# SimplySnap/torchPDLP

Measured on AMD Instinct MI355X. Metric: PDHG iterations/sec, higher is better.
Workload: dtype f32; 1 GPU; synthetic random feasible LP 10000000x10000000, 100 nnz/row (density 1.0e-05), gen_lp recipe 'box' seed 0; nnz=1000000000, primal_weight_update=True, parallelism=single GPU

## Files before the change

### include/pdlp_hip.h

```cpp
#ifndef PDLP_HIP_H
#define PDLP_HIP_H

#include <stdint.h>

#ifdef __cplusplus
extern "C" {
#endif

#define PDLP_OK 0
#define PDLP_ERR_INVALID (-1)
#define PDLP_ERR_WORKSPACE (-2)
#define PDLP_ERR_STATE (-3)
#define PDLP_ERR_COMM (-4)
#define PDLP_ERR_HIP_BASE (-1000)

enum { PDLP_F32 = 0, PDLP_F64 = 1, PDLP_MIXED = 2 };

enum { PDLP_CUR = 0, PDLP_AVG = 1, PDLP_PREV = 2 };

enum {
    PDLP_BUF_X_CUR = 0, PDLP_BUF_X_PREV = 1, PDLP_BUF_XBAR = 2, PDLP_BUF_X_AVG = 3,
    PDLP_BUF_Y_CUR = 4, PDLP_BUF_Y_PREV = 5, PDLP_BUF_Y_AVG = 6,
    PDLP_BUF_RED = 7,
    PDLP_BUF_X_SUM = 8, PDLP_BUF_Y_SUM = 9,
// ... 38 lines not shown
    const int32_t* tile_ptr;
    const int64_t* blk_base;
    const uint32_t* cnt;
    int32_t rem_rows_n, rem_segs_n;
    const int32_t* rem_rows;
    const int32_t* rem_rptr;
    const int32_t* rem_sptr;
    const int32_t* rem_col;
    const void* rem_val;
    void* rem_work;
    void* rem_extra;
    void* rem_extra_f32;
} pdlp_tiles;

typedef struct pdlp_solver* pdlp_handle;

const char* pdlp_strerror(int code);
int pdlp_abi_version(void);

int pdlp_workspace_bytes(const pdlp_problem* p, int64_t* bytes);
int pdlp_create(pdlp_handle* out, const pdlp_problem* p, void* workspace, int64_t workspace_bytes);
void pdlp_destroy(pdlp_handle h);
int pdlp_attach_tiles(pdlp_handle h, int transpose, const pdlp_tiles* t);
int pdlp_schedule_info(pdlp_handle h, int transpose, int32_t* nblk, const int64_t** blocks);
int pdlp_attach_sorted(pdlp_handle h, int transpose, const uint32_t* sidx, const void* sval, const int32_t* cbase);
int pdlp_buffer_ptr(pdlp_handle h, int which, void** ptr);

int pdlp_set_iterate(pdlp_handle h, const void* x_local, const void* y_local);
int pdlp_get_iterate(pdlp_handle h, int which, void* x_local, void* y_local);
int pdlp_set_step(pdlp_handle h, double eta, double omega, double theta, int64_t iteration);
int pdlp_set_omega(pdlp_handle h, double omega);
int pdlp_get_scalars(pdlp_handle h, double out[PDLP_NSCAL]);

int pdlp_primal_half(pdlp_handle h, int adaptive);
int pdlp_dual_half(pdlp_handle h, int adaptive);
int pdlp_primal_half_begin(pdlp_handle h);
int pdlp_dual_half_begin(pdlp_handle h, int adaptive);
int pdlp_split_info(pdlp_handle h, int transpose, int32_t out[4]);
int pdlp_tile_limits(pdlp_handle h, int32_t out[6]);
int pdlp_adaptive_retry(pdlp_handle h);
int pdlp_adaptive_reduce(pdlp_handle h);
int pdlp_adaptive_update(pdlp_handle h);
int pdlp_iterate(pdlp_handle h, int iters, int adaptive);
int pdlp_fixed_advance(pdlp_handle h, int iters);
int pdlp_halpern_iterate(pdlp_handle h, int iters);

// ... 119 lines not shown
```

### torchpdlp_amd/_native.py

```python
from __future__ import annotations

import ctypes as C
import os

_HERE = os.path.dirname(os.path.abspath(__file__))
LIB_PATH = os.environ.get("PDLP_LIB") or os.path.join(_HERE, "libpdlp_hip.so")

ABI_VERSION = 18
PDLP_F32, PDLP_F64, PDLP_MIXED = 0, 1, 2
CUR, AVG, PREV = 0, 1, 2
(BUF_X_CUR, BUF_X_PREV, BUF_XBAR, BUF_X_AVG, BUF_Y_CUR, BUF_Y_PREV, BUF_Y_AVG, BUF_RED, BUF_X_SUM, BUF_Y_SUM,
 BUF_SCALARS, BUF_DX, BUF_DY, BUF_LAM_PREV, BUF_GDX, BUF_GDY) = range(16)
NRED, NSCAL = 8, 16
OPT_RUNNING_KKT, OPT_KTY_REUSE, OPT_GRAPH, OPT_SPLIT_SLOTS, OPT_PRODUCER_PIECES, OPT_BEGIN_INLINE, OPT_PEER_EXCHANGE, OPT_PEER_TIMEOUT_MS, OPT_PEER_LOCAL_FIRST, OPT_PEER_PUSH = range(10)
PEER_INFO_BYTES, PEER_LOOPBACK, PEER_LOOPBACK_HOST = 256, 1, 2
S_ETA, S_OMEGA, S_THETA, S_TAU, S_SIGMA, S_WPEND, S_ETASUM, S_K, S_INV1PT, S_ACCEPT, S_ETABAR, S_DEN, S_ETASUM_PREV = range(13)


class PdlpProblem(C.Structure):
    _fields_ = [("dtype", C.c_int32), ("device", C.c_int32), ("m", C.c_int64), ("n", C.c_int64), ("m_ineq", C.c_int64),
                ("row0", C.c_int64), ("row1", C.c_int64), ("col0", C.c_int64), ("col1", C.c_int64),
                ("K_rowptr", C.c_void_p), ("K_colidx", C.c_void_p), ("K_val", C.c_void_p),
                ("KT_rowptr", C.c_void_p), ("KT_colidx", C.c_void_p), ("KT_val", C.c_void_p),
                ("c", C.c_void_p), ("l", C.c_void_p), ("u", C.c_void_p), ("q", C.c_void_p),
# ... 18 lines not shown
                ("dy", C.c_void_p),
                ("eta", C.c_void_p), ("omega", C.c_void_p), ("eta_sum", C.c_void_p), ("wpend", C.c_void_p),
                ("live", C.c_void_p), ("action", C.c_void_p), ("part", C.c_void_p), ("out", C.c_void_p)]


class PdlpBatchFeed(C.Structure):
    _fields_ = [("N", C.c_int32), ("c", C.c_void_p), ("q", C.c_void_p), ("l", C.c_void_p), ("u", C.c_void_p),
                ("x0", C.c_void_p), ("y0", C.c_void_p), ("K_val", C.c_void_p), ("KT_val", C.c_void_p),
                ("eta", C.c_void_p), ("omega", C.c_void_p)]


BATCH_PART_PER_COL = 2 * 4 * 8192


_H = C.c_void_p
_I, _I64, _D, _P = C.c_int, C.c_int64, C.c_double, C.c_void_p
SIGNATURES = {
    "pdlp_strerror": (C.c_char_p, [_I]),
    "pdlp_abi_version": (_I, []),
    "pdlp_workspace_bytes": (_I, [C.POINTER(PdlpProblem), C.POINTER(_I64)]),
    "pdlp_create": (_I, [C.POINTER(_H), C.POINTER(PdlpProblem), _P, _I64]),
    "pdlp_destroy": (None, [_H]),
    "pdlp_attach_tiles": (_I, [_H, _I, C.POINTER(PdlpTiles)]),
    "pdlp_schedule_info": (_I, [_H, _I, C.POINTER(C.c_int32), C.POINTER(_P)]),
    "pdlp_attach_sorted": (_I, [_H, _I, _P, _P, _P]),
    "pdlp_buffer_ptr": (_I, [_H, _I, C.POINTER(_P)]),
    "pdlp_set_iterate": (_I, [_H, _P, _P]),
    "pdlp_get_iterate": (_I, [_H, _I, _P, _P]),
    "pdlp_set_step": (_I, [_H, _D, _D, _D, _I64]),
    "pdlp_set_omega": (_I, [_H, _D]),
    "pdlp_get_scalars": (_I, [_H, C.POINTER(_D)]),
    "pdlp_primal_half": (_I, [_H, _I]),
    "pdlp_dual_half": (_I, [_H, _I]),
    "pdlp_primal_half_piece": (_I, [_H, _I, _I, _I]),
    "pdlp_dual_half_piece": (_I, [_H, _I, _I, _I]),
    "pdlp_primal_half_begin": (_I, [_H]),
    "pdlp_dual_half_begin": (_I, [_H, _I]),
    "pdlp_split_info": (_I, [_H, _I, C.POINTER(C.c_int32)]),
    "pdlp_tile_limits": (_I, [_H, C.POINTER(C.c_int32)]),
    "pdlp_adaptive_retry": (_I, [_H]),
    "pdlp_adaptive_reduce": (_I, [_H]),
    "pdlp_adaptive_update": (_I, [_H]),
    "pdlp_iterate": (_I, [_H, _I, _I]),
    "pdlp_halpern_iterate": (_I, [_H, _I]),
    "pdlp_set_row_upper": (_I, [_H, _P]),
    "pdlp_set_exchange_chunks": (_I, [_H, _I]),
# ... 117 lines not shown
```

### torchpdlp_amd/csrc/pdlp_handle.inc

```
namespace {

struct Schedule {
    int64_t* blk = nullptr;
    uint32_t* rplo = nullptr;
    int nblk = 0;
    int grid = 0;
    int64_t* lch = nullptr;
    int32_t* lrow = nullptr;
    int32_t* lptr = nullptr;
    void* longpart = nullptr;
    int nchunks = 0, nlong = 0, lgrid = 0;
    const uint32_t* sidx = nullptr;
    const void* sval = nullptr;
    const int32_t* cbase = nullptr;
    bool tiled = false;
    pdlp_tiles t{};
    int loc_pa = 0, loc_pb = 0;
    int slotsA = 0, slotsB = 0;
    bool pending = false;
    bool pending_inline = false;
    int32_t* ptab = nullptr;
    int64_t ptab_cap = 0;
    int nphase = 0;
    int ph_off[MAX_PHASE] = {0}, ph_cnt[MAX_PHASE] = {0}, ph_slots[MAX_PHASE] = {0}, ph_slot0[MAX_PHASE] = {0};
    int64_t sb[MAX_PHASE] = {0};
    int chunks_done = 0;
    int nrange = 0;
    int rb_lo[MAX_PHASE] = {0};
};

inline int64_t max_blocks(int64_t rows, int64_t nnz) { return 2 * (rows / ROWS_CAP + nnz / NNZ_CAP) + 4; }

inline int64_t max_chunks(int64_t nnz) { return 2 * (nnz / NNZ_CAP) + 2; }
inline int64_t max_long(int64_t nnz) { return nnz / NNZ_CAP + 1; }
constexpr int LONG_GRID = 64;

inline int64_t rowsum_groups(int64_t rows)
{
    if (rows <= (int64_t)512 * 40 * 128) return 32;
// ... 267 lines not shown
```

### torchpdlp_amd/csrc/pdlp_hip.hip

```cpp
#include <hip/hip_runtime.h>
#include <rccl/rccl.h>
#include <dlfcn.h>
#include <unistd.h>

#include <cmath>
#include <cstdint>
#include <cstdio>
#include <cstdlib>
#include <cstring>
#include <new>
#include <type_traits>
#include <vector>

#include "pdlp_hip.h"

namespace {

constexpr int BLOCK = 256;
constexpr int NNZ_CAP = 2048;
constexpr int ROWS_CAP = 256;
constexpr int MAX_GRID = 2048;
constexpr int NACC = 4;
constexpr int MAX_CHUNKS = 4;
constexpr int MAX_PHASE = MAX_CHUNKS + 2;
// ... 165 lines not shown
        case PDLP_BUF_X_AVG: *ptr = h->xb[h->ix_avg]; break;
        case PDLP_BUF_Y_CUR: *ptr = h->yb[h->ix_cur]; break;
        case PDLP_BUF_Y_PREV: *ptr = h->yb[h->ix_prev]; break;
        case PDLP_BUF_Y_AVG: *ptr = h->yb[h->ix_avg]; break;
        case PDLP_BUF_RED: *ptr = h->red; break;
        case PDLP_BUF_X_SUM: *ptr = h->x_sum; break;
        case PDLP_BUF_Y_SUM: *ptr = h->y_sum; break;
        case PDLP_BUF_SCALARS: *ptr = h->sc; break;
        case PDLP_BUF_DX: *ptr = h->dxf; break;
        case PDLP_BUF_DY: *ptr = h->dyf; break;
        case PDLP_BUF_LAM_PREV: *ptr = h->lam_prev; break;
        case PDLP_BUF_GDX: if (!h->mixed) return PDLP_ERR_STATE; *ptr = h->gdx; break;
        case PDLP_BUF_GDY: if (!h->mixed) return PDLP_ERR_STATE; *ptr = h->gdy; break;
        default: return PDLP_ERR_INVALID;
    }
    return PDLP_OK;
}

int pdlp_attach_tiles(pdlp_handle h, int transpose, const pdlp_tiles* t)
{
    if (!h) return PDLP_ERR_INVALID;
    Schedule& s = transpose ? h->sKT : h->sK;
    drop_graphs(h);
    if (!t) { s.tiled = false; return configure_split(h, transpose != 0); }
    const int64_t rows = transpose ? h->nl : h->ml;
    const int rpt_max = h->p.dtype == PDLP_F64 ? TileCfg<double, double>::RPT_MAX : TileCfg<float, float>::RPT_MAX;
    const int cap_max = h->p.dtype == PDLP_F64 ? TileCfg<double, double>::CAP : TileCfg<float, float>::CAP;
    if (t->rpt < 1 || t->rpt > rpt_max || t->cap > cap_max || t->lw < 4 || (((uint64_t)t->cap + 8u) << t->lw) > (1ull << 32)) return PDLP_ERR_INVALID;
    const int64_t rb = (int64_t)TNT * t->rpt;
    if (t->nblk != (int)((rows + rb - 1) / rb) || t->npanel < 1) return PDLP_ERR_INVALID;
    if (t->groups < 1 || t->groups > h->rs_groups || t->groups > t->npanel) return PDLP_ERR_INVALID;
    if (t->nblk > h->part_blocks) return PDLP_ERR_INVALID;
    if (!t->idx || !t->val || !t->tile_ptr || !t->blk_base || !t->cnt) return PDLP_ERR_INVALID;
    if (((uintptr_t)t->idx & 15u) || ((uintptr_t)t->val & 15u) || ((uintptr_t)t->cnt & 15u)) return PDLP_ERR_INVALID;
    if (t->rem_rows_n < 0 || t->rem_segs_n < t->rem_rows_n) return PDLP_ERR_INVALID;
    if (t->rem_rows_n > 0 && (!t->rem_rows || !t->rem_rptr || !t->rem_sptr || !t->rem_col || !t->rem_val || !t->rem_work || !t->rem_extra ||
                              (h->mixed && !t->rem_extra_f32)))
        return PDLP_ERR_INVALID;
    s.t = *t;
    s.tiled = true;
    return configure_split(h, transpose != 0);
}

int pdlp_schedule_info(pdlp_handle h, int transpose, int32_t* nblk, const int64_t** blocks)
{
    if (!h || !nblk || !blocks) return PDLP_ERR_INVALID;
    const Schedule& s = transpose ? h->sKT : h->sK;
    *nblk = s.nblk;
    *blocks = s.blk;
    return PDLP_OK;
}

int pdlp_attach_sorted(pdlp_handle h, int transpose, const uint32_t* sidx, const void* sval, const int32_t* cbase)
{
    if (!h) return PDLP_ERR_INVALID;
    if ((sidx == nullptr) != (sval == nullptr) || (sidx == nullptr) != (cbase == nullptr)) return PDLP_ERR_INVALID;
    Schedule& s = transpose ? h->sKT : h->sK;
    drop_graphs(h);
    s.sidx = sidx; s.sval = sval; s.cbase = cbase;
    return PDLP_OK;
}

int pdlp_set_iterate(pdlp_handle h, const void* x_local, const void* y_local)
{
// ... 376 lines not shown
```

### torchpdlp_amd/csrc/pdlp_kernel_tiled.inc

```
#ifndef PDLP_PRIO_P1
#define PDLP_PRIO_P1 3
#define PDLP_PRIO_P2 0
#endif
#ifndef PDLP_GROUP_FAST
#define PDLP_GROUP_FAST 1
#endif
#ifndef PDLP_EPI_GROUP
#define PDLP_EPI_GROUP 0
#endif
#ifndef PDLP_TNT
#define PDLP_TNT 512
#endif
constexpr int TNT = PDLP_TNT;
typedef unsigned int u32x4 __attribute__((ext_vector_type(4)));
typedef float f32x4 __attribute__((ext_vector_type(4)));
typedef double f64x4 __attribute__((ext_vector_type(4)));
#ifndef PDLP_F32_RPT
#define PDLP_F32_RPT 40
#define PDLP_F32_CAP 16384
#define PDLP_F32_TU 4
#endif
template <typename T, typename TV> struct TileCfg;
template <> struct TileCfg<float, float> { static constexpr int RPT_MAX = PDLP_F32_RPT, CAP = PDLP_F32_CAP, TU = PDLP_F32_TU, MINW = 4; typedef f32x4 V4; };
template <> struct TileCfg<double, double> { static constexpr int RPT_MAX = 24, CAP = 8192, TU = 2, MINW = 4; typedef f64x4 V4; };
template <> struct TileCfg<double, float> { static constexpr int RPT_MAX = PDLP_F32_RPT, CAP = PDLP_F32_CAP > 16384 ? 16384 : PDLP_F32_CAP, TU = 2, MINW = 2; typedef f32x4 V4; };
constexpr int TRPT_MAX_ANY = PDLP_F32_RPT > 40 ? PDLP_F32_RPT : 40;

__device__ __forceinline__ float fma_t(float a, float b, float c) { return __builtin_fmaf(a, b, c); }
__device__ __forceinline__ double fma_t(double a, double b, double c) { return __builtin_fma(a, b, c); }
__device__ __forceinline__ float clamp01_t(float x) { return __builtin_amdgcn_fmed3f(x, 0.0f, 1.0f); }
__device__ __forceinline__ double clamp01_t(double x) { return __builtin_fmin(__builtin_fmax(x, 0.0), 1.0); }

template <typename T, typename TV, class Epi, bool FUSED>
__global__ __launch_bounds__(TNT, (TileCfg<T, TV>::MINW)) void k_tiled_fused(const uint32_t* __restrict__ tidx, const TV* __restrict__ tval,
                                                        const int32_t* __restrict__ tile_ptr, const int64_t* __restrict__ blk_base,
                                                        const uint32_t* __restrict__ tcnt,
                                                        int npanel, int lw, int rpt, int nrows, int nblk,
                                                        int vtotal, const int32_t* __restrict__ ptab, int slot0, int b0, int nbl,
                                                        const T* __restrict__ vin, T* __restrict__ rowsum,
                                                        int64_t rs_stride, const T* __restrict__ extra, Epi epi,
                                                        double* __restrict__ partials)
{
    typedef TileCfg<T, TV> Cfg;
    constexpr int TRPT_MAX = Cfg::RPT_MAX, TCW = TRPT_MAX / 8, TCAP = Cfg::CAP, TU = Cfg::TU;
    constexpr int TGRP = TNT * 4 * TU;
    typedef typename Cfg::V4 V4;
    __shared__ __attribute__((aligned(16))) T prod[TCAP + 8];
    __shared__ int wsum[TNT / 64];
    __shared__ double dred8[TNT / 64];
    const int tid = threadIdx.x, lane = tid & 63, wv = tid >> 6;
    const int ngrp = FUSED ? 1 : (int)(gridDim.x / (unsigned)nbl);
#if PDLP_GROUP_FAST
    const int b = FUSED ? blockIdx.x : b0 + (int)(blockIdx.x / (unsigned)ngrp);
    const int grp = FUSED ? 0 : (int)(blockIdx.x % (unsigned)ngrp);
#else
    const int b = FUSED ? blockIdx.x : b0 + (int)(blockIdx.x % (unsigned)nbl);
    const int grp = FUSED ? 0 : (int)(blockIdx.x / (unsigned)nbl);
#endif
    const int p_lo = (int)((int64_t)grp * vtotal / ngrp), p_hi = (int)((int64_t)(grp + 1) * vtotal / ngrp);
    auto pmap = [&](int v) { return ptab ? ptab[v] : v; };
    const uint32_t mask = (1u << lw) - 1u;
    if (FUSED) epi.load();
    T acc[TRPT_MAX];
#pragma unroll
    for (int r = 0; r < TRPT_MAX; ++r) acc[r] = (T)0;

    const uint32_t trash = (uint32_t)TCAP << lw;
    tidx += blk_base[b];
    tval += blk_base[b];
    auto load_into = [&](u32x4 (&pk)[TU], V4 (&vv)[TU], int g0, int i1) {
#pragma unroll
        for (int u = 0; u < TU; ++u) {
            const int i = g0 + (u * TNT + tid) * 4;
            if (i < i1) {
                pk[u] = __builtin_nontemporal_load(reinterpret_cast<const u32x4*>(tidx + i));
                vv[u] = __builtin_nontemporal_load(reinterpret_cast<const V4*>(tval + i));
            } else {
                pk[u] = u32x4{trash, trash, trash, trash};
                vv[u] = V4{(TV)0, (TV)0, (TV)0, (TV)0};
            }
        }
    };
#ifndef PDLP_ROUND
#define PDLP_ROUND 4
#endif
    auto consume = [&](u32x4 (&pk)[TU], V4 (&vv)[TU], int g0, int i1, const T* __restrict__ xin) {
        constexpr int RPC = 4 / PDLP_ROUND, NR = TU * RPC;
        T xg[TU * 4];
        bool on[TU];
#pragma unroll
        for (int u = 0; u < TU; ++u) on[u] = g0 + (u * TNT + __builtin_amdgcn_readfirstlane(wv) * 64) * 4 < i1;
        auto pkw = [&](int u, int k) -> uint32_t { return k == 0 ? pk[u].x : k == 1 ? pk[u].y : k == 2 ? pk[u].z : pk[u].w; };
        auto vvw = [&](int u, int k) -> TV { return k == 0 ? vv[u].x : k == 1 ? vv[u].y : k == 2 ? vv[u].z : vv[u].w; };
        auto products = [&](int r) {
            const int u = r / RPC, k0 = (r % RPC) * PDLP_ROUND;
            if (on[u]) {
#pragma unroll
                for (int k = k0; k < k0 + PDLP_ROUND; ++k) prod[pkw(u, k) >> lw] = (T)vvw(u, k) * xg[4 * u + k];
            }
        };
#pragma unroll
        for (int r = 0; r < NR; ++r) {
            const int u = r / RPC, k0 = (r % RPC) * PDLP_ROUND;
            if (r > 0) { products(r - 1); __builtin_amdgcn_sched_barrier(0); }
            if (on[u]) {
#pragma unroll
                for (int k = k0; k < k0 + PDLP_ROUND; ++k) {
                    xg[4 * u + k] = *reinterpret_cast<const T*>(reinterpret_cast<const char*>(xin) + ((pkw(u, k) & mask) * (uint32_t)sizeof(T)));
                }
            }
            __builtin_amdgcn_sched_barrier(0);
        }
        products(NR - 1);
    };
    const size_t tile0 = (size_t)b * npanel;
    const size_t tp0 = (size_t)b * (npanel + 1);
    const bool has_panels = p_lo < vtotal;
    const size_t ntiles = (size_t)nblk * npanel;
    auto load_counts = [&](uint32_t (&cwd)[TCW], size_t tile) {
        const u32x4 a = __builtin_nontemporal_load(reinterpret_cast<const u32x4*>(tcnt) + tile * TNT + tid);
        cwd[0] = a.x;
        if (TCW > 1) cwd[1 < TCW ? 1 : 0] = a.y;
        if (TCW > 2) cwd[2 < TCW ? 2 : 0] = a.z;
        if (TCW > 3) cwd[3 < TCW ? 3 : 0] = a.w;
#pragma unroll
        for (int q = 4; q < TCW; ++q) cwd[q] = __builtin_nontemporal_load(tcnt + ntiles * TNT * 4 + (tile * (TCW > 4 ? TCW - 4 : 1) + (q - 4)) * TNT + tid);
    };
    u32x4 pk[TU];
    V4 vv[TU];
    int i0 = has_panels ? tile_ptr[tp0 + pmap(p_lo)] : 0;
    int i1 = has_panels ? tile_ptr[tp0 + pmap(p_lo) + 1] : 0;
    load_into(pk, vv, i0, i1);

    for (int i = tid; i < TCAP + 8; i += TNT) prod[i] = (T)0;
    __syncthreads();
    uint32_t cwn[TCW];
    {
        load_counts(cwn, tile0 + (has_panels ? pmap(p_lo) : 0));
    }
    for (int v = p_lo; v < p_hi; ++v) {
        const int p = pmap(v);
        const T* __restrict__ xin = vin + ((size_t)p << lw);
        int i0n = i1, i1n = i1;
        if (v + 1 < p_hi) {
            const int pn = pmap(v + 1);
            i0n = tile_ptr[tp0 + pn];
            i1n = tile_ptr[tp0 + pn + 1];
        }
        uint32_t cw[TCW];
        uint32_t total = 0;
#pragma unroll
        for (int q = 0; q < TCW; ++q) cw[q] = cwn[q];
#pragma unroll
        for (int q = 0; q < TCW; ++q) {
            const uint32_t n2 = (cw[q] & 0x0f0f0f0fu) + ((cw[q] >> 4) & 0x0f0f0f0fu);
            total += (n2 * 0x01010101u) >> 24;
        }
        total = wave_incl_scan_u32(total);
        if (lane == 63) wsum[wv] = (int)total;
        __builtin_amdgcn_s_setprio(PDLP_PRIO_P1);
        for (int g0 = i0; g0 < i1; g0 += TGRP) {
            consume(pk, vv, g0, i1, xin);
            if (g0 + TGRP < i1) load_into(pk, vv, g0 + TGRP, i1);
            else load_into(pk, vv, i0n, i1n);
        }
        if (i0 >= i1) load_into(pk, vv, i0n, i1n);
        {
            load_counts(cwn, tile0 + (v + 1 < p_hi ? pmap(v + 1) : p));
        }
        __builtin_amdgcn_s_setprio(PDLP_PRIO_P2);
        __syncthreads();
        int sb = 0;
#pragma unroll
        for (int w = 0; w < TNT / 64; ++w) sb += (w < wv) ? wsum[w] : 0;
        uint32_t sbase = (uint32_t)__builtin_amdgcn_readfirstlane(sb);
#pragma unroll
        for (int q = 0; q < TCW; ++q) {
            if (8 * q < rpt) {
                uint32_t cE = cw[q] & 0x0f0f0f0fu, cO = (cw[q] >> 4) & 0x0f0f0f0fu;
                asm("" : "+v"(cE), "+v"(cO));
                uint32_t sE = cE, sO = cO;
                wave_incl_scan2_u32(sE, sO);
                const uint32_t tE = (uint32_t)__builtin_amdgcn_readlane((int)sE, 63), tO = (uint32_t)__builtin_amdgcn_readlane((int)sO, 63);
                const uint32_t eE = sE - cE, eO = sO - cO;
                constexpr int RG = sizeof(T) == 8 ? 2 : 4;
#pragma unroll
                for (int g = 0; g < 8 / RG; ++g) {
                    if (8 * q + RG * g < rpt) {
                        int cc[RG], oo[RG];
// ... 111 lines not shown
        for (int g0 = 0; g0 < groups; g0 += 4) {
            T part[4];
#pragma unroll
            for (int k = 0; k < 4; ++k) {
                const int g = g0 + k < glast ? g0 + k : glast;
                part[k] = __builtin_nontemporal_load(rowsum + (size_t)g * rs_stride + row);
            }
            s = g0 == 0 ? part[0] : s + part[0];
#pragma unroll
            for (int k = 1; k < 4; ++k) s = g0 + k < groups ? s + part[k] : s;
        }
        if (extra) s += extra[row];
        epi(row, s, pre, acc);
    }
    if (Epi::NA > 0) {
#pragma unroll
        for (int r = 0; r < Epi::NA; ++r) {
            const double v = block_sum(acc[r], dred);
            if (threadIdx.x == 0) partials[(size_t)blockIdx.x * NACC + r] = v;
        }
    }
}

template <typename T, typename TV>
__global__ __launch_bounds__(BLOCK) void k_rem_segments(int ns, const int32_t* __restrict__ sptr, const int32_t* __restrict__ col,
                                                        const TV* __restrict__ val, const T* __restrict__ vin, T* __restrict__ seg_sum)
{
    const int lt = threadIdx.x & 7;
    const int64_t stride = ((int64_t)gridDim.x * BLOCK) >> 3;
    const int64_t ns_pad = ((int64_t)ns + stride - 1) / stride * stride;
    for (int64_t g = ((int64_t)blockIdx.x * BLOCK + threadIdx.x) >> 3; g < ns_pad; g += stride) {
        T s = (T)0;
        if (g < ns) {
            const int a = sptr[g], nn = sptr[g + 1] - a;
            const int last = nn - 1;
            for (int i0 = lt; i0 < nn; i0 += 64) {
                T lv[8], lg[8];
                int lc[8];
#pragma unroll
                for (int u = 0; u < 8; ++u) {
                    const int i = i0 + 8 * u, ic = i < last ? i : last;
                    lv[u] = (T)val[a + ic];
                    lc[u] = col[a + ic];
                }
#pragma unroll
                for (int u = 0; u < 8; ++u) lg[u] = vin[lc[u]];
// ... 49 lines not shown
```

### torchpdlp_amd/csrc/pdlp_products.inc

```
namespace {

template <typename T, typename TV>
void launch_tiled_groups(pdlp_handle h, const Schedule& s, int rows, const void* vin, hipStream_t stream, int vgroups, int vtotal,
                         const int32_t* ptab, int slot0, int b0 = 0, int nbl = -1)
{
    if (nbl < 0) nbl = s.t.nblk - b0;
    if (vtotal <= 0 || vgroups <= 0 || nbl <= 0) return;
    const int groups = vgroups < vtotal ? vgroups : vtotal;
    StoreEpi<T> none{nullptr};
    hipLaunchKernelGGL((k_tiled_fused<T, TV, StoreEpi<T>, false>), dim3(nbl * groups), dim3(TNT), 0, stream, s.t.idx,
                       (const TV*)s.t.val, s.t.tile_ptr, s.t.blk_base, s.t.cnt, s.t.npanel, s.t.lw, s.t.rpt, rows, s.t.nblk, vtotal, ptab,
                       slot0, b0, nbl, (const T*)vin, (T*)h->rowsum, h->rs_stride, (const T*)nullptr, none, (double*)nullptr);
}

template <typename T, typename TV>
void launch_phase(pdlp_handle h, const Schedule& s, int rows, const void* vin, hipStream_t stream, int phase, int b0 = 0, int nbl = -1)
{
    launch_tiled_groups<T, TV>(h, s, rows, vin, stream, s.ph_slots[phase], s.ph_cnt[phase], s.ptab + s.ph_off[phase], s.ph_slot0[phase], b0, nbl);
}

template <typename T, typename TV, class Epi>
int launch_mat(pdlp_handle h, bool transpose, const void* vin, Epi epi, double* partials)
{
    if (!h->use_split && (h->sK.pending || h->sKT.pending)) {
        if (!(h->sK.pending ? h->sK.pending_inline : h->sKT.pending_inline)) HIP_TRY(hipStreamWaitEvent(h->stream, h->ev_out, 0));
        h->sK.pending = h->sKT.pending = false;
        h->sK.chunks_done = h->sKT.chunks_done = 0;
    }
    const Schedule& s = transpose ? h->sKT : h->sK;
    if (s.nblk == 0) return PDLP_OK;
    if (s.tiled) {
        const int rows = (int)(transpose ? h->nl : h->ml);
        const T* extra = nullptr;
        if (s.t.rem_rows_n > 0 && h->range_sel > 0) {
            extra = (const T*)(sizeof(T) == 4 && h->es == 8 ? s.t.rem_extra_f32 : s.t.rem_extra);
        } else if (s.t.rem_rows_n > 0) {
            T* ex = (T*)(sizeof(T) == 4 && h->es == 8 ? s.t.rem_extra_f32 : s.t.rem_extra);
            hipLaunchKernelGGL((k_rem_segments<T, TV>), dim3(grid_for((int64_t)s.t.rem_segs_n * 8)), dim3(BLOCK), 0, h->stream, s.t.rem_segs_n,
                               s.t.rem_sptr, s.t.rem_col, (const TV*)s.t.rem_val, (const T*)vin, (T*)s.t.rem_work);
            hipLaunchKernelGGL((k_rem_rows<T>), dim3(grid_for((int64_t)s.t.rem_rows_n * 8)), dim3(BLOCK), 0, h->stream, s.t.rem_rows_n, s.t.rem_rows,
                               s.t.rem_rptr, (const T*)s.t.rem_work, ex);
            extra = ex;
        }
        if (s.t.groups == 1 && !(s.pending && h->use_split)) {
            hipLaunchKernelGGL((k_tiled_fused<T, TV, Epi, true>), dim3(s.t.nblk), dim3(TNT), 0, h->stream, s.t.idx, (const TV*)s.t.val,
                               s.t.tile_ptr, s.t.blk_base, s.t.cnt, s.t.npanel, s.t.lw, s.t.rpt, rows, s.t.nblk, s.t.npanel,
                               (const int32_t*)nullptr, 0, 0, s.t.nblk, (const T*)vin, (T*)h->rowsum, h->rs_stride, extra, epi, partials);
        } else if (s.pending && h->use_split) {
            Schedule& sm = transpose ? h->sKT : h->sK;
            const int R = s.nrange > 1 ? s.nrange : 1, last = s.nphase - 1;
            const int r_from = h->range_sel < 0 ? 0 : h->range_sel, r_to = h->range_sel < 0 ? R : h->range_sel + 1;
            if (r_from == 0) {
                for (int ph = 1 + sm.chunks_done; ph < (R > 1 ? last : s.nphase); ++ph) launch_phase<T, TV>(h, s, rows, vin, h->stream, ph);
                sm.chunks_done = 0;
            }
            int pofs = 0;
            for (int r = 0; r < r_from && R > 1; ++r) pofs += range_epi_grid(s, r, rows);
            for (int r = r_from; r < r_to && r < R; ++r) {
                if (R > 1) launch_phase<T, TV>(h, s, rows, vin, h->stream, last, s.rb_lo[r], s.rb_lo[r + 1] - s.rb_lo[r]);
                if (r == 0 && !s.pending_inline) HIP_TRY(hipStreamWaitEvent(h->stream, h->ev_out, 0));
                const int lo = R > 1 ? range_rows_lo(s, r) : 0, hi = R > 1 ? range_rows_hi(s, r, rows) : rows;
                if (hi > lo)
                    hipLaunchKernelGGL((k_rowsum_epilogue<T, Epi>), dim3(grid_for(hi - lo)), dim3(BLOCK), 0, h->stream, (const T*)h->rowsum,
                                       s.slotsA + s.slotsB, h->rs_stride, hi, extra, epi, partials + (size_t)pofs * NACC, lo);
                pofs += R > 1 ? range_epi_grid(s, r, rows) : 0;
            }
        } else {
            launch_tiled_groups<T, TV>(h, s, rows, vin, h->stream, s.t.groups, s.t.npanel, (const int32_t*)nullptr, 0);
            hipLaunchKernelGGL((k_rowsum_epilogue<T, Epi>), dim3(grid_for(rows)), dim3(BLOCK), 0, h->stream, (const T*)h->rowsum,
                               s.t.groups, h->rs_stride, rows, extra, epi, partials);
// ... 220 lines not shown
```

### torchpdlp_amd/engine_kernels.py

```python
from __future__ import annotations

import ctypes as C
from typing import Optional

import torch

from . import _native as N
from . import tiled as _tiled

TILED_MIN_NNZ = 1 << 20
TILED_MIN_COLS = 1 << 16
TILED_MIN_PER_ROW = 10


def wants_tiles(mode: str, rows: int, cols: int, nnz: int) -> bool:
    if mode == "0" or rows == 0 or (mode != "1" and (cols < TILED_MIN_COLS or nnz < TILED_MIN_NNZ)):
        return False
    return not (mode == "auto" and nnz < TILED_MIN_PER_ROW * rows)


class KernelChoice:

    def tile_limits(self) -> dict:
        out = (C.c_int32 * 6)()
        N.check(self.lib.pdlp_tile_limits(self.h, out), "pdlp_tile_limits")
        return dict(max_groups=out[0], max_blocks=out[1], rpt_max=out[2], cap=out[3], nt=out[4])

    def _maybe_attach_tiles(self):
        kn = self.knobs
        mode = kn.tiled if self._want_tiles else "0"
        self.kernels = ["csr", "csr"]
        if kn.sorted == "1" and self._want_tiles:
            for transpose in (0, 1):
                self.attach_sorted(transpose)
        if mode == "0":
# ... 59 lines not shown

    def attach_tiles(self, transpose: int, t: Optional["_tiled.Tiles"]):
        if t is None:
            N.check(self.lib.pdlp_attach_tiles(self.h, int(transpose), None), "pdlp_attach_tiles")
            self._plans = {}
            self.tiles[int(transpose)] = None
            self.kernels[int(transpose)] = "csr"
            return
        rem = [0, 0] + [None] * 8
        if t.nrem:
            rows = self.nl if transpose else self.ml
            t._work = torch.empty(int(t.rem_sptr.numel()) - 1, dtype=torch.float64, device=self.device)
            t._extra = torch.zeros(rows, dtype=self.dtype, device=self.device)
            t._extra32 = torch.zeros(rows, dtype=torch.float32, device=self.device) if self.mixed else None
            rem = [int(t.rem_rows.numel()), int(t.rem_sptr.numel()) - 1, t.rem_rows.data_ptr(), t.rem_rptr.data_ptr(), t.rem_sptr.data_ptr(),
                   t.rem_col.data_ptr(), t.rem_val.data_ptr(), t._work.data_ptr(), t._extra.data_ptr(),
                   None if t._extra32 is None else t._extra32.data_ptr()]
        rel, base = t.abi_tile_ptr()
        desc = N.PdlpTiles(t.lw, t.rpt, t.cap, t.nblk, t.npanel, t.groups, t.idx.data_ptr(), t.val.data_ptr(), rel.data_ptr(), base.data_ptr(),
                           t.cnt.data_ptr(), *rem)
        N.check(self.lib.pdlp_attach_tiles(self.h, int(transpose), C.byref(desc)), "pdlp_attach_tiles")
        self._plans = {}
        self.tiles[int(transpose)] = t
        self.kernels[int(transpose)] = ("tiled" if t.groups == 1 else f"tiled/{t.groups} groups") + (f" + remainder {t.nrem}" if t.nrem else "")
```

### torchpdlp_amd/tiled.py

```python
from __future__ import annotations

import os
from dataclasses import dataclass, field
from typing import Optional

import torch

LW_DEFAULT = 16
NT = 512
RPT_MAX = 40
CAP = 16384
RPT_MAX_F64 = 24
CAP_F64 = 8192
GROUP = 256
NCU = 512
LMAX = 15
GMAX = 255
SEG = 512


@dataclass
class Tiles:
    lw: int
    rpt: int
# ... 332 lines not shown
        prod[slots] = val[i0:i1].double() * xd[cols]
        ends = torch.cumsum(counts, 0)
        csum = torch.cat([torch.zeros(1, dtype=torch.float64, device=x.device), torch.cumsum(prod[:int(ends[-1])], 0)])
        y[b * RB:(b + 1) * RB] += csum[ends] - csum[ends - counts]

    idx = t.idx.long() & 0xFFFFFFFF
    tp = t.tile_ptr.long().tolist()
    for b in range(t.nblk):
        for p in range(t.npanel):
            tile = b * t.npanel + p
            i0, i1 = tp[tile], tp[tile + 1]
            pk = idx[i0:i1]
            one(pk >> t.lw, t.val, torch.clamp(p * W + (pk & (W - 1)), max=t.ncols - 1), i0, i1, tile_row_counts(t, tile), b)
    if t.nrem:
        sp, rptr = t.rem_sptr.long(), t.rem_rptr.long().tolist()
        prod = t.rem_val.double() * xd[t.rem_col.long()]
        cs = torch.cat([torch.zeros(1, dtype=torch.float64, device=x.device), torch.cumsum(prod, 0)])
        seg = cs[sp[1:]] - cs[sp[:-1]]
        for i, r in enumerate(t.rem_rows.tolist()):
            y[r] += seg[rptr[i]:rptr[i + 1]].sum()
    return y[:t.nrows]


SORTED_MAX_ITEMS = 2048
SORTED_COL_BITS = 21
SORTED_DENSE_GAP = 32.0
SORTED_MIN_SHARE = 0.5


def sorted_row_blocks(first: torch.Tensor, colidx: torch.Tensor, val: torch.Tensor, force: bool = True):
    nb, nnz = int(first.numel()) - 1, int(val.numel())
    first = first.long()
    lens = first[1:] - first[:-1]
    dev = colidx.device
    bid = torch.repeat_interleave(torch.arange(nb, device=dev), lens)
    cl = colidx.long()
    big = torch.iinfo(torch.int64).max
    cmin = torch.full((nb,), big, dtype=torch.int64, device=dev).scatter_reduce_(0, bid, cl, "amin")
    cmax = torch.full((nb,), -1, dtype=torch.int64, device=dev).scatter_reduce_(0, bid, cl, "amax")
    ok = (lens > 0) & (lens <= SORTED_MAX_ITEMS) & (cmax - cmin < (1 << SORTED_COL_BITS))
    if not force:
        gap = (cmax - cmin).double() / (lens - 1).clamp(min=1).double()
        dense = ok & (gap < SORTED_DENSE_GAP)
        if float(lens[dense].sum()) < SORTED_MIN_SHARE * nnz:
            return None
    order = torch.argsort((bid << 32) | cl, stable=True)
# ... 6 lines not shown
```

Measured before the change: 283.1 iterations/s.

## Pack tiled SpMV item indices into 24-bit entries with per-run column bases

Adds a float32-only packed format for tiled SpMV items. Each 32-bit index (slot<<lw | col) is recoded as a 24-bit word: a 14-bit slot plus a 10-bit column offset from a per-64-item-run 16-bit base. The bases are read once per wave and broadcast with readlane. This cuts index traffic from 4 to 3 bytes per nonzero, lowering total bytes per nnz from about 8 to 7 in this memory-bound kernel. The cost is extra ALU work to unpack (alignbit and readlane), unaligned 12-byte loads, a one-time pack kernel at attach time, and a fallback to 32-bit items when a run spans more than 1023 columns.

```diff
diff --git a/include/pdlp_hip.h b/include/pdlp_hip.h
--- a/include/pdlp_hip.h
+++ b/include/pdlp_hip.h
@@ -84,6 +84,8 @@
 int pdlp_create(pdlp_handle* out, const pdlp_problem* p, void* workspace, int64_t workspace_bytes);
 void pdlp_destroy(pdlp_handle h);
 int pdlp_attach_tiles(pdlp_handle h, int transpose, const pdlp_tiles* t);
+int pdlp_pack_tile_items(const uint32_t* idx, int64_t items, int lw, uint32_t* idx24, uint32_t* run_base, int32_t* flag, void* stream);
+int pdlp_attach_packed_items(pdlp_handle h, int transpose, const uint32_t* idx24, const uint32_t* run_base);
 int pdlp_schedule_info(pdlp_handle h, int transpose, int32_t* nblk, const int64_t** blocks);
 int pdlp_attach_sorted(pdlp_handle h, int transpose, const uint32_t* sidx, const void* sval, const int32_t* cbase);
 int pdlp_buffer_ptr(pdlp_handle h, int which, void** ptr);
diff --git a/torchpdlp_amd/_native.py b/torchpdlp_amd/_native.py
--- a/torchpdlp_amd/_native.py
+++ b/torchpdlp_amd/_native.py
@@ -64,6 +64,8 @@
     "pdlp_create": (_I, [C.POINTER(_H), C.POINTER(PdlpProblem), _P, _I64]),
     "pdlp_destroy": (None, [_H]),
     "pdlp_attach_tiles": (_I, [_H, _I, C.POINTER(PdlpTiles)]),
+    "pdlp_pack_tile_items": (_I, [_P, _I64, _I, _P, _P, _P, _P]),
+    "pdlp_attach_packed_items": (_I, [_H, _I, _P, _P]),
     "pdlp_schedule_info": (_I, [_H, _I, C.POINTER(C.c_int32), C.POINTER(_P)]),
     "pdlp_attach_sorted": (_I, [_H, _I, _P, _P, _P]),
     "pdlp_buffer_ptr": (_I, [_H, _I, C.POINTER(_P)]),
diff --git a/torchpdlp_amd/csrc/pdlp_handle.inc b/torchpdlp_amd/csrc/pdlp_handle.inc
--- a/torchpdlp_amd/csrc/pdlp_handle.inc
+++ b/torchpdlp_amd/csrc/pdlp_handle.inc
@@ -15,6 +15,8 @@
     const int32_t* cbase = nullptr;
     bool tiled = false;
     pdlp_tiles t{};
+    const uint32_t* idx24 = nullptr;
+    const uint32_t* run_base = nullptr;
     int loc_pa = 0, loc_pb = 0;
     int slotsA = 0, slotsB = 0;
     bool pending = false;
diff --git a/torchpdlp_amd/csrc/pdlp_hip.hip b/torchpdlp_amd/csrc/pdlp_hip.hip
--- a/torchpdlp_amd/csrc/pdlp_hip.hip
+++ b/torchpdlp_amd/csrc/pdlp_hip.hip
@@ -211,6 +211,7 @@
     if (!h) return PDLP_ERR_INVALID;
     Schedule& s = transpose ? h->sKT : h->sK;
     drop_graphs(h);
+    s.idx24 = s.run_base = nullptr;
     if (!t) { s.tiled = false; return configure_split(h, transpose != 0); }
     const int64_t rows = transpose ? h->nl : h->ml;
     const int rpt_max = h->p.dtype == PDLP_F64 ? TileCfg<double, double>::RPT_MAX : TileCfg<float, float>::RPT_MAX;
@@ -229,6 +230,36 @@
     s.t = *t;
     s.tiled = true;
     return configure_split(h, transpose != 0);
+}
+
+int pdlp_pack_tile_items(const uint32_t* idx, int64_t items, int lw, uint32_t* idx24, uint32_t* run_base, int32_t* flag, void* stream)
+{
+    if (!idx || !idx24 || !run_base || !flag || items < 0 || (items & 255) || lw < 4 || lw > 16) return PDLP_ERR_INVALID;
+    if (((uintptr_t)idx & 15u) || ((uintptr_t)idx24 & 3u) || ((uintptr_t)run_base & 3u) || ((uintptr_t)flag & 3u)) return PDLP_ERR_INVALID;
+    hipStream_t st = (hipStream_t)stream;
+    const int64_t nchunks = items >> 8;
+    HIP_TRY(hipMemsetAsync(flag, 0, sizeof(int32_t), st));
+    HIP_TRY(hipMemsetAsync(run_base + nchunks * 2, 0, (size_t)P24_BASE_TAIL * 8, st));
+    if (nchunks > 0) {
+        hipLaunchKernelGGL(k_pack_items24, dim3(grid_for(nchunks * 64)), dim3(BLOCK), 0, st, idx, nchunks, lw, idx24, run_base, flag);
+        HIP_TRY(hipGetLastError());
+    }
+    return PDLP_OK;
+}
+
+int pdlp_attach_packed_items(pdlp_handle h, int transpose, const uint32_t* idx24, const uint32_t* run_base)
+{
+    if (!h || (idx24 == nullptr) != (run_base == nullptr)) return PDLP_ERR_INVALID;
+    Schedule& s = transpose ? h->sKT : h->sK;
+    if (idx24) {
+        if (!s.tiled || h->p.dtype != PDLP_F32) return PDLP_ERR_STATE;
+        if (s.t.cap > (1 << P24_SLOT_BITS) || s.t.lw > 16 || ((uintptr_t)idx24 & 3u) || ((uintptr_t)run_base & 3u)) return PDLP_ERR_INVALID;
+    }
+    if (s.pending) return PDLP_ERR_STATE;
+    drop_graphs(h);
+    s.idx24 = idx24;
+    s.run_base = run_base;
+    return PDLP_OK;
 }
 
 int pdlp_schedule_info(pdlp_handle h, int transpose, int32_t* nblk, const int64_t** blocks)
diff --git a/torchpdlp_amd/csrc/pdlp_kernel_tiled.inc b/torchpdlp_amd/csrc/pdlp_kernel_tiled.inc
--- a/torchpdlp_amd/csrc/pdlp_kernel_tiled.inc
+++ b/torchpdlp_amd/csrc/pdlp_kernel_tiled.inc
@@ -31,10 +31,12 @@
 __device__ __forceinline__ float clamp01_t(float x) { return __builtin_amdgcn_fmed3f(x, 0.0f, 1.0f); }
 __device__ __forceinline__ double clamp01_t(double x) { return __builtin_fmin(__builtin_fmax(x, 0.0), 1.0); }
 
-template <typename T, typename TV, class Epi, bool FUSED>
+constexpr int P24_COL_BITS = 10, P24_SLOT_BITS = 14;
+constexpr int P24_BASE_TAIL = TNT * 4 * TileCfg<float, float>::TU / 256;
+template <typename T, typename TV, class Epi, bool FUSED, bool PACKED = false>
 __global__ __launch_bounds__(TNT, (TileCfg<T, TV>::MINW)) void k_tiled_fused(const uint32_t* __restrict__ tidx, const TV* __restrict__ tval,
                                                         const int32_t* __restrict__ tile_ptr, const int64_t* __restrict__ blk_base,
-                                                        const uint32_t* __restrict__ tcnt,
+                                                        const uint32_t* __restrict__ tcnt, const uint32_t* __restrict__ trb,
                                                         int npanel, int lw, int rpt, int nrows, int nblk,
                                                         int vtotal, const int32_t* __restrict__ ptab, int slot0, int b0, int nbl,
                                                         const T* __restrict__ vin, T* __restrict__ rowsum,
@@ -66,17 +68,33 @@
     for (int r = 0; r < TRPT_MAX; ++r) acc[r] = (T)0;
 
     const uint32_t trash = (uint32_t)TCAP << lw;
-    tidx += blk_base[b];
+    static_assert(!PACKED || (sizeof(T) == 4 && sizeof(TV) == 4 && TCAP <= (1 << P24_SLOT_BITS)), "packed items: float32 tiles only");
+    tidx += PACKED ? (blk_base[b] >> 2) * 3 : blk_base[b];
     tval += blk_base[b];
-    auto load_into = [&](u32x4 (&pk)[TU], V4 (&vv)[TU], int g0, int i1) {
+    static_assert(!PACKED || TU == 4, "packed items: lane l holds bases of chunk (l >> 1) & 3");
+    if (PACKED) trb += (blk_base[b] >> 8) * 2;
+    auto load_into = [&](u32x4 (&pk)[TU], V4 (&vv)[TU], uint32_t& rbv, int g0, int i1) {
+        uint32_t gq = (uint32_t)g0 >> 2;
+        if (PACKED) {
+            asm volatile("" : "+s"(gq));
+            const uint32_t ob = ((((gq >> 6) + ((lane >> 1) & (TU - 1)) * (TNT / 64) + wv) << 1) + (lane & 1)) << 2;
+            rbv = *reinterpret_cast<const uint32_t*>(reinterpret_cast<const char*>(trb) + ob);
+        }
 #pragma unroll
         for (int u = 0; u < TU; ++u) {
             const int i = g0 + (u * TNT + tid) * 4;
             if (i < i1) {
-                pk[u] = __builtin_nontemporal_load(reinterpret_cast<const u32x4*>(tidx + i));
-                vv[u] = __builtin_nontemporal_load(reinterpret_cast<const V4*>(tval + i));
+                if (PACKED) {
+                    const uint32_t i4 = gq + (uint32_t)(u * TNT + tid);
+                    const uint32_t* __restrict__ q = reinterpret_cast<const uint32_t*>(reinterpret_cast<const char*>(tidx) + i4 * 12u);
+                    pk[u] = u32x4{__builtin_nontemporal_load(q), __builtin_nontemporal_load(q + 1), __builtin_nontemporal_load(q + 2), 0u};
+                    vv[u] = __builtin_nontemporal_load(reinterpret_cast<const V4*>(reinterpret_cast<const char*>(tval) + i4 * 16u));
+                } else {
+                    pk[u] = __builtin_nontemporal_load(reinterpret_cast<const u32x4*>(tidx + i));
+                    vv[u] = __builtin_nontemporal_load(reinterpret_cast<const V4*>(tval + i));
+                }
             } else {
-                pk[u] = u32x4{trash, trash, trash, trash};
+                pk[u] = PACKED ? u32x4{0u, 0u, 0u, 0u} : u32x4{trash, trash, trash, trash};
                 vv[u] = V4{(TV)0, (TV)0, (TV)0, (TV)0};
             }
         }
@@ -84,19 +102,26 @@
 #ifndef PDLP_ROUND
 #define PDLP_ROUND 4
 #endif
-    auto consume = [&](u32x4 (&pk)[TU], V4 (&vv)[TU], int g0, int i1, const T* __restrict__ xin) {
+    auto consume = [&](u32x4 (&pk)[TU], V4 (&vv)[TU], uint32_t rbv, int g0, int i1, const T* __restrict__ xin) {
         constexpr int RPC = 4 / PDLP_ROUND, NR = TU * RPC;
         T xg[TU * 4];
         bool on[TU];
 #pragma unroll
         for (int u = 0; u < TU; ++u) on[u] = g0 + (u * TNT + __builtin_amdgcn_readfirstlane(wv) * 64) * 4 < i1;
-        auto pkw = [&](int u, int k) -> uint32_t { return k == 0 ? pk[u].x : k == 1 ? pk[u].y : k == 2 ? pk[u].z : pk[u].w; };
+        auto pkw = [&](int u, int k) -> uint32_t {
+            if (PACKED)
+                return k == 0 ? pk[u].x : k == 1 ? __builtin_amdgcn_alignbit(pk[u].y, pk[u].x, 24)
+                              : k == 2 ? __builtin_amdgcn_alignbit(pk[u].z, pk[u].y, 16) : pk[u].z >> 8;
+            return k == 0 ? pk[u].x : k == 1 ? pk[u].y : k == 2 ? pk[u].z : pk[u].w;
+        };
+        auto rbw = [&](int u, int k) -> uint32_t { return ((uint32_t)__builtin_amdgcn_readlane((int)rbv, 2 * u + (k >> 1)) >> (16 * (k & 1))) & 0xffffu; };
+        auto slot = [&](int u, int k) -> uint32_t { return PACKED ? (pkw(u, k) >> P24_COL_BITS) & ((1u << P24_SLOT_BITS) - 1u) : pkw(u, k) >> lw; };
         auto vvw = [&](int u, int k) -> TV { return k == 0 ? vv[u].x : k == 1 ? vv[u].y : k == 2 ? vv[u].z : vv[u].w; };
         auto products = [&](int r) {
             const int u = r / RPC, k0 = (r % RPC) * PDLP_ROUND;
             if (on[u]) {
 #pragma unroll
-                for (int k = k0; k < k0 + PDLP_ROUND; ++k) prod[pkw(u, k) >> lw] = (T)vvw(u, k) * xg[4 * u + k];
+                for (int k = k0; k < k0 + PDLP_ROUND; ++k) prod[slot(u, k)] = (T)vvw(u, k) * xg[4 * u + k];
             }
         };
 #pragma unroll
@@ -106,7 +131,11 @@
             if (on[u]) {
 #pragma unroll
                 for (int k = k0; k < k0 + PDLP_ROUND; ++k) {
-                    xg[4 * u + k] = *reinterpret_cast<const T*>(reinterpret_cast<const char*>(xin) + ((pkw(u, k) & mask) * (uint32_t)sizeof(T)));
+                    if (PACKED)
+                        xg[4 * u + k] = *reinterpret_cast<const T*>(reinterpret_cast<const char*>(xin + rbw(u, k)) +
+                                                                    ((pkw(u, k) << 2) & (((1u << P24_COL_BITS) - 1u) << 2)));
+                    else
+                        xg[4 * u + k] = *reinterpret_cast<const T*>(reinterpret_cast<const char*>(xin) + ((pkw(u, k) & mask) * (uint32_t)sizeof(T)));
                 }
             }
             __builtin_amdgcn_sched_barrier(0);
@@ -127,10 +156,11 @@
         for (int q = 4; q < TCW; ++q) cwd[q] = __builtin_nontemporal_load(tcnt + ntiles * TNT * 4 + (tile * (TCW > 4 ? TCW - 4 : 1) + (q - 4)) * TNT + tid);
     };
     u32x4 pk[TU];
+    uint32_t rbv = 0;
     V4 vv[TU];
     int i0 = has_panels ? tile_ptr[tp0 + pmap(p_lo)] : 0;
     int i1 = has_panels ? tile_ptr[tp0 + pmap(p_lo) + 1] : 0;
-    load_into(pk, vv, i0, i1);
+    load_into(pk, vv, rbv, i0, i1);
 
     for (int i = tid; i < TCAP + 8; i += TNT) prod[i] = (T)0;
     __syncthreads();
@@ -160,11 +190,11 @@
         if (lane == 63) wsum[wv] = (int)total;
         __builtin_amdgcn_s_setprio(PDLP_PRIO_P1);
         for (int g0 = i0; g0 < i1; g0 += TGRP) {
-            consume(pk, vv, g0, i1, xin);
-            if (g0 + TGRP < i1) load_into(pk, vv, g0 + TGRP, i1);
-            else load_into(pk, vv, i0n, i1n);
-        }
-        if (i0 >= i1) load_into(pk, vv, i0n, i1n);
+            consume(pk, vv, rbv, g0, i1, xin);
+            if (g0 + TGRP < i1) load_into(pk, vv, rbv, g0 + TGRP, i1);
+            else load_into(pk, vv, rbv, i0n, i1n);
+        }
+        if (i0 >= i1) load_into(pk, vv, rbv, i0n, i1n);
         {
             load_counts(cwn, tile0 + (v + 1 < p_hi ? pmap(v + 1) : p));
         }
@@ -322,6 +352,43 @@
     }
 }
 
+__global__ __launch_bounds__(BLOCK) void k_pack_items24(const uint32_t* __restrict__ idx, int64_t nchunks, int lw, uint32_t* __restrict__ idx24,
+                                                        uint32_t* __restrict__ run_base, int32_t* __restrict__ flag)
+{
+    const int lane = threadIdx.x & 63;
+    const uint32_t mask = (1u << lw) - 1u;
+    const int64_t stride = (int64_t)gridDim.x * (BLOCK / 64);
+    for (int64_t c = (int64_t)blockIdx.x * (BLOCK / 64) + (threadIdx.x >> 6); c < nchunks; c += stride) {
+        const u32x4 w4 = *(reinterpret_cast<const u32x4*>(idx) + c * 64 + lane);
+        const uint32_t w[4] = {w4.x, w4.y, w4.z, w4.w};
+        const uint32_t last = (uint32_t)__builtin_amdgcn_readlane((int)w4.w, 63);
+        const bool has_pad = (last & mask) == 0u;
+        uint32_t f[4], rb[4];
+        bool bad = false;
+#pragma unroll
+        for (int j = 0; j < 4; ++j) {
+            const bool pad = has_pad && w[j] == last;
+            const uint32_t col = w[j] & mask, sl = w[j] >> lw;
+            uint32_t m = pad ? 0xffffffffu : col;
+#pragma unroll
+            for (int off = 32; off > 0; off >>= 1) {
+                const uint32_t o = (uint32_t)__shfl_xor((int)m, off, 64);
+                m = o < m ? o : m;
+            }
+            rb[j] = m == 0xffffffffu ? 0u : m;
+            const uint32_t d = pad ? 0u : col - rb[j];
+            bad = bad || d >= (1u << P24_COL_BITS) || sl >= (1u << P24_SLOT_BITS);
+            f[j] = ((sl & ((1u << P24_SLOT_BITS) - 1u)) << P24_COL_BITS) | (d & ((1u << P24_COL_BITS) - 1u));
+        }
+        uint32_t* __restrict__ o = idx24 + (c * 64 + lane) * 3;
+        o[0] = f[0] | (f[1] << 24);
+        o[1] = (f[1] >> 8) | (f[2] << 16);
+        o[2] = (f[2] >> 16) | (f[3] << 8);
+        if (lane < 2) run_base[c * 2 + lane] = lane ? rb[2] | (rb[3] << 16) : rb[0] | (rb[1] << 16);
+        if (bad) *flag = 1;
+    }
+}
+
 template <typename T, typename TV>
 __global__ __launch_bounds__(BLOCK) void k_rem_segments(int ns, const int32_t* __restrict__ sptr, const int32_t* __restrict__ col,
                                                         const TV* __restrict__ val, const T* __restrict__ vin, T* __restrict__ seg_sum)
diff --git a/torchpdlp_amd/csrc/pdlp_products.inc b/torchpdlp_amd/csrc/pdlp_products.inc
--- a/torchpdlp_amd/csrc/pdlp_products.inc
+++ b/torchpdlp_amd/csrc/pdlp_products.inc
@@ -8,9 +8,18 @@
     if (vtotal <= 0 || vgroups <= 0 || nbl <= 0) return;
     const int groups = vgroups < vtotal ? vgroups : vtotal;
     StoreEpi<T> none{nullptr};
+    if constexpr (std::is_same<T, float>::value && std::is_same<TV, float>::value) {
+        if (s.idx24) {
+            hipLaunchKernelGGL((k_tiled_fused<T, TV, StoreEpi<T>, false, true>), dim3(nbl * groups), dim3(TNT), 0, stream, s.idx24,
+                               (const TV*)s.t.val, s.t.tile_ptr, s.t.blk_base, s.t.cnt, s.run_base, s.t.npanel, s.t.lw, s.t.rpt, rows, s.t.nblk,
+                               vtotal, ptab, slot0, b0, nbl, (const T*)vin, (T*)h->rowsum, h->rs_stride, (const T*)nullptr, none, (double*)nullptr);
+            return;
+        }
+    }
     hipLaunchKernelGGL((k_tiled_fused<T, TV, StoreEpi<T>, false>), dim3(nbl * groups), dim3(TNT), 0, stream, s.t.idx,
-                       (const TV*)s.t.val, s.t.tile_ptr, s.t.blk_base, s.t.cnt, s.t.npanel, s.t.lw, s.t.rpt, rows, s.t.nblk, vtotal, ptab,
-                       slot0, b0, nbl, (const T*)vin, (T*)h->rowsum, h->rs_stride, (const T*)nullptr, none, (double*)nullptr);
+                       (const TV*)s.t.val, s.t.tile_ptr, s.t.blk_base, s.t.cnt, (const uint32_t*)nullptr, s.t.npanel, s.t.lw, s.t.rpt, rows,
+                       s.t.nblk, vtotal, ptab, slot0, b0, nbl, (const T*)vin, (T*)h->rowsum, h->rs_stride, (const T*)nullptr, none,
+                       (double*)nullptr);
 }
 
 template <typename T, typename TV>
@@ -43,9 +52,18 @@
             extra = ex;
         }
         if (s.t.groups == 1 && !(s.pending && h->use_split)) {
-            hipLaunchKernelGGL((k_tiled_fused<T, TV, Epi, true>), dim3(s.t.nblk), dim3(TNT), 0, h->stream, s.t.idx, (const TV*)s.t.val,
-                               s.t.tile_ptr, s.t.blk_base, s.t.cnt, s.t.npanel, s.t.lw, s.t.rpt, rows, s.t.nblk, s.t.npanel,
-                               (const int32_t*)nullptr, 0, 0, s.t.nblk, (const T*)vin, (T*)h->rowsum, h->rs_stride, extra, epi, partials);
+            bool packed = false;
+            if constexpr (std::is_same<T, float>::value && std::is_same<TV, float>::value) {
+                if ((packed = s.idx24 != nullptr))
+                    hipLaunchKernelGGL((k_tiled_fused<T, TV, Epi, true, true>), dim3(s.t.nblk), dim3(TNT), 0, h->stream, s.idx24, (const TV*)s.t.val,
+                                       s.t.tile_ptr, s.t.blk_base, s.t.cnt, s.run_base, s.t.npanel, s.t.lw, s.t.rpt, rows, s.t.nblk, s.t.npanel,
+                                       (const int32_t*)nullptr, 0, 0, s.t.nblk, (const T*)vin, (T*)h->rowsum, h->rs_stride, extra, epi, partials);
+            }
+            if (!packed)
+                hipLaunchKernelGGL((k_tiled_fused<T, TV, Epi, true>), dim3(s.t.nblk), dim3(TNT), 0, h->stream, s.t.idx, (const TV*)s.t.val,
+                                   s.t.tile_ptr, s.t.blk_base, s.t.cnt, (const uint32_t*)nullptr, s.t.npanel, s.t.lw, s.t.rpt, rows, s.t.nblk,
+                                   s.t.npanel, (const int32_t*)nullptr, 0, 0, s.t.nblk, (const T*)vin, (T*)h->rowsum, h->rs_stride, extra, epi,
+                                   partials);
         } else if (s.pending && h->use_split) {
             Schedule& sm = transpose ? h->sKT : h->sK;
             const int R = s.nrange > 1 ? s.nrange : 1, last = s.nphase - 1;
diff --git a/torchpdlp_amd/engine_kernels.py b/torchpdlp_amd/engine_kernels.py
--- a/torchpdlp_amd/engine_kernels.py
+++ b/torchpdlp_amd/engine_kernels.py
@@ -1,6 +1,7 @@
 from __future__ import annotations
 
 import ctypes as C
+import os
 from typing import Optional
 
 import torch
@@ -11,6 +12,11 @@
 TILED_MIN_NNZ = 1 << 20
 TILED_MIN_COLS = 1 << 16
 TILED_MIN_PER_ROW = 10
+PACKED_ITEMS_DEFAULT = True
+
+
+def packed_items_mode(env=None) -> str:
+    return (os.environ if env is None else env).get("PDLP_PACKED_ITEMS", "auto") or "auto"
 
 
 def wants_tiles(mode: str, rows: int, cols: int, nnz: int) -> bool:
@@ -116,4 +122,38 @@
         N.check(self.lib.pdlp_attach_tiles(self.h, int(transpose), C.byref(desc)), "pdlp_attach_tiles")
         self._plans = {}
         self.tiles[int(transpose)] = t
-        self.kernels[int(transpose)] = ("tiled" if t.groups == 1 else f"tiled/{t.groups} groups") + (f" + remainder {t.nrem}" if t.nrem else "")
+        packed = self._maybe_attach_packed_items(int(transpose), t)
+        self.kernels[int(transpose)] = ("tiled" if t.groups == 1 else f"tiled/{t.groups} groups") + (f" + remainder {t.nrem}" if t.nrem else "") + \
+            (", 32-bit items" if self._packed_items_apply() and not packed else "")
+
+    def _packed_items_apply(self) -> bool:
+        return self.dtype == torch.float32 and not self.mixed
+
+    def _maybe_attach_packed_items(self, transpose: int, t: "_tiled.Tiles") -> bool:
+        mode = packed_items_mode()
+        want = self._packed_items_apply() and (mode == "1" or (mode != "0" and PACKED_ITEMS_DEFAULT))
+        packed = False
+        if want and not _tiled.packed_items_shape_ok(t):
+            if mode == "1":
+                raise N.PdlpError(f"PDLP_PACKED_ITEMS=1: the tile set does not qualify (cap {t.cap}, lw {t.lw}, or a row block of 2^30 items)")
+        elif want:
+            idx24 = torch.empty(t.items // 4 * 3, dtype=torch.int32, device=self.device)
+            run_base = torch.empty(2 * (t.items // _tiled.GROUP + _tiled.P24_TAIL), dtype=torch.int32, device=self.device)
+            flag = torch.empty(1, dtype=torch.int32, device=self.device)
+            torch.cuda.current_stream(self.device).synchronize()
+            N.check(self.lib.pdlp_pack_tile_items(t.idx.data_ptr(), t.items, t.lw, idx24.data_ptr(), run_base.data_ptr(), flag.data_ptr(),
+                                                  self.stream.cuda_stream), "pdlp_pack_tile_items")
+            self.stream.synchronize()
+            if int(flag.item()) == 0:
+                N.check(self.lib.pdlp_attach_packed_items(self.h, transpose, idx24.data_ptr(), run_base.data_ptr()), "pdlp_attach_packed_items")
+                t._idx24, t._run_base = idx24, run_base
+                packed = True
+            elif mode == "1":
+                raise N.PdlpError("PDLP_PACKED_ITEMS=1: a run of 64 sorted items spans more than 1023 columns")
+        if not packed:
+            t._idx24 = t._run_base = None
+        nnz = max(int(t.stats.get("tiled", t.items)), 1)
+        extra = int(t._run_base.numel()) * 4 if packed else 0
+        t.stats["packed_items"] = packed
+        t.stats["bytes_per_nnz"] = (t.items * (7 if packed else 8) + extra + int(t.cnt.numel()) * 4) / nnz
+        return packed
diff --git a/torchpdlp_amd/tiled.py b/torchpdlp_amd/tiled.py
--- a/torchpdlp_amd/tiled.py
+++ b/torchpdlp_amd/tiled.py
@@ -378,6 +378,63 @@
     return y[:t.nrows]
 
 
+P24_COL_BITS = 10
+P24_SLOT_BITS = 14
+P24_TAIL = 32
+
+
+def packed_items_shape_ok(t: Tiles) -> bool:
+    if t.val.dtype != torch.float32 or t.cap > (1 << P24_SLOT_BITS) or t.lw > 16:
+        return False
+    return t.items == 0 or int(t.abi_tile_ptr()[0].max()) < 2 ** 30
+
+
+def pack_items24(t: Tiles):
+    if t.lw > 16:
+        raise ValueError("run bases are 16-bit: lw <= 16")
+    dev = t.idx.device
+    w = (t.idx.long() & 0xFFFFFFFF).view(-1, 64, 4)
+    mask = (1 << t.lw) - 1
+    last = w[:, 63, 3].view(-1, 1, 1)
+    pad = ((last & mask) == 0) & (w == last)
+    col, sl = w & mask, w >> t.lw
+    big = 1 << 32
+    m = torch.where(pad, big, col).amin(dim=1) if w.numel() else col.new_zeros((0, 4))
+    rb = torch.where(m == big, 0, m)
+    d = torch.where(pad, 0, col - rb.view(-1, 1, 4))
+    fits = not bool(((d >= (1 << P24_COL_BITS)) | (sl >= (1 << P24_SLOT_BITS))).any())
+    f = ((sl & ((1 << P24_SLOT_BITS) - 1)) << P24_COL_BITS) | (d & ((1 << P24_COL_BITS) - 1))
+    by = torch.stack([f & 255, (f >> 8) & 255, (f >> 16) & 255], dim=-1).to(torch.uint8)
+    idx24 = by.reshape(-1).view(torch.int32) if by.numel() else torch.zeros(0, dtype=torch.int32, device=dev)
+    rbw = torch.stack([rb[:, 0] | (rb[:, 1] << 16), rb[:, 2] | (rb[:, 3] << 16)], dim=-1)
+    run_base = torch.cat([_wrap_i32(rbw.reshape(-1)), torch.zeros(2 * P24_TAIL, dtype=torch.int32, device=dev)])
+    return idx24, run_base, fits
+
+
+def tile_item_counts(t: Tiles) -> torch.Tensor:
+    ntiles = t.nblk * t.npanel
+    n4 = ntiles * t.nt * 4
+    w = torch.cat([t.cnt[:n4].view(ntiles, -1), t.cnt[n4:].view(ntiles, -1)], dim=1).long() & 0xFFFFFFFF
+    shifts = (torch.arange(8, device=w.device) * 4).view(1, 1, 8)
+    return ((w.unsqueeze(-1) >> shifts) & 15).sum((1, 2))
+
+
+def unpack_items24(idx24: torch.Tensor, run_base: torch.Tensor, t: Tiles) -> torch.Tensor:
+    by = idx24.view(torch.uint8).long().view(-1, 64, 4, 3)
+    f = by[..., 0] | (by[..., 1] << 8) | (by[..., 2] << 16)
+    nch = f.shape[0]
+    rbw = run_base[:2 * nch].long().view(-1, 2) & 0xFFFFFFFF
+    rb = torch.stack([rbw[:, 0] & 0xFFFF, rbw[:, 0] >> 16, rbw[:, 1] & 0xFFFF, rbw[:, 1] >> 16], dim=-1)
+    tp = t.tile_ptr.long()
+    tile_of_chunk = torch.repeat_interleave(torch.arange(tp.numel() - 1, device=tp.device), (tp[1:] - tp[:-1]) // GROUP)
+    first = tp[:-1][tile_of_chunk] // GROUP
+    pos = ((torch.arange(nch, device=tp.device) - first) * GROUP).view(-1, 1, 1) + \
+        torch.arange(64, device=tp.device).view(1, 64, 1) + 64 * torch.arange(4, device=tp.device).view(1, 1, 4)
+    real = pos < tile_item_counts(t)[tile_of_chunk].view(-1, 1, 1)
+    col = torch.where(real, rb.view(-1, 1, 4) + (f & ((1 << P24_COL_BITS) - 1)), 0)
+    return _wrap_i32(((f >> P24_COL_BITS) << t.lw) | col).reshape(-1)
+
+
 SORTED_MAX_ITEMS = 2048
 SORTED_COL_BITS = 21
 SORTED_DENSE_GAP = 32.0
```

Measured after the change: 289.7 iterations/s (median of 6 runs). 2.3% higher.
